# pierric/smart-chess-rust

Measured on AMD Instinct MI355X. Metric: MCTS simulations/sec (whole node), self-play rollout=180, at 1/2/4/8 MI355X, higher is better.
Workload: dtype bf16

## Files before the change

### smart-chess-rust_amd/csrc/mcts_kernels.hip

```cpp
#include "search_expand.hpp"

#include "launchers.hpp"

namespace sc {
__global__ __launch_bounds__(64) void k_debug_find_max(const float* u, int n, int* out) {
    const int lane = threadIdx.x;
    if (n <= 64) {
        const int r = wave_argmax_last_lane(lane < n ? u[lane] : 0.f, lane < n);
        if (lane == 0) out[0] = r;
    } else if (lane == 0) {
        out[0] = -2;
    }
    float best_u = 0.f;
    int best_i = -1;
#pragma unroll
    for (int r = 0; r < 4; r++) {
        const int i = lane + 64 * r;
        if (i < n) {
            const float v = u[i];
            if (best_i < 0 || v >= best_u) {
                best_u = v;
                best_i = i;
            }
        }
    }
    const int r4 = wave_argmax_last(best_u, best_i);
    if (lane == 0) out[1] = r4;
}

__global__ __launch_bounds__(64) void k_synth_eval(SpParams p) {
    const int g = blockIdx.x, lane = threadIdx.x;
    GameCtl& c = p.ctl[g];
    if (c.status != ST_ACTIVE || c.leaf_kind != LK_EVAL) return;
    const Position& pos = p.tpos[(size_t)g * p.tpos_cap + c.n_exp];
    uint64_t h = synth_pos_hash(pos) ^ p.synth_salt;
    int n = c.n_legal;
    const uint16_t* lm = p.legal_mv + (size_t)g * MAXC;
    if (p.evaluator == SYNTH_UNIFORM) {
        for (int i = lane; i < n; i += 64) p.prior[(size_t)g * MAXC + i] = 1.0f / (float)n;
        if (lane == 0) p.value[g] = 0.0f;
        return;
    }
    const bool coarse = p.evaluator == SYNTH_COARSE;
    unsigned long long sum = 0;
    for (int i = lane; i < n; i += 64) sum += coarse ? 1u + (synth_weight(h, lm[i]) >> 22) : synth_weight(h, lm[i]);
    sum = scw::wave_sum_u64(sum);
    float fs = (float)sum;
    for (int i = lane; i < n; i += 64)
        p.prior[(size_t)g * MAXC + i] = (float)(coarse ? 1u + (synth_weight(h, lm[i]) >> 22) : synth_weight(h, lm[i])) / fs;
    if (lane == 0) {
        const float v = synth_value(h);
        p.value[g] = coarse ? (v < -0.5f ? -0.5f : v >= 0.5f ? 0.5f : 0.0f) : v;
    }
}

__device__ inline int match_white(const SpParams& p, unsigned long long k) { return p.match_colours ? (int)(k & 1) : 0; }
__device__ inline unsigned long long match_ordinal(SpParams& p, int lane, int side) {
    const unsigned long long total = (unsigned long long)p.total_games;
    if (!p.match_colours && side) return total;
    unsigned long long n = 0;
    if (lane == 0) n = atomicAdd(&p.cnt->match_next[side], 1ULL);
    n = __shfl(n, 0, 64);
    const unsigned long long k = p.match_colours ? 2ULL * n + (unsigned long long)side : n;
    return k < total ? k : total;
}
__device__ inline int match_line_of(const SpParams& p, const MatchLines& ln, unsigned long long k) {
    return (int)((p.match_colours ? k >> 1 : k) % (unsigned long long)ln.n);
}
__device__ inline void match_copy_line(SpParams& p, int g, int lane, const Position* line, int len) {
    constexpr int W = (int)(sizeof(Position) / 8);
    static_assert(sizeof(Position) % 8 == 0, "a record is copied in 8-byte words");
    const unsigned long long* src = reinterpret_cast<const unsigned long long*>(line);
    unsigned long long* hist = reinterpret_cast<unsigned long long*>(p.hist + (size_t)g * p.hist_cap);
    unsigned long long* root = reinterpret_cast<unsigned long long*>(p.tpos + (size_t)g * p.tpos_cap);
    const int words = (len + 1) * W;
    wave_sync();
    for (int i = lane; i < words; i += 64) hist[i] = src[i];
    if (lane < W) root[lane] = src[len * W + lane];
    if (lane == 0) {
        p.ctl[g].ply = len;
        p.ctl[g].start_ply = len;
    }
}
__device__ inline void match_slot_start(SpParams& p, const MatchLines& ln, int g, int lane) {
    GameCtl& c = p.ctl[g];
    const int st = c.status, side = p.match_side & 1;
    const unsigned long long total = (unsigned long long)p.total_games;
    unsigned long long k;
    if (st == ST_MATCH_WAIT) {
        k = c.game_id - p.first_game_id;
    } else if (st == ST_IDLE) {
        k = match_ordinal(p, lane, side);
        if (k >= total) k = match_ordinal(p, lane, side ^ 1);
        if (k >= total) return;
    } else {
        return;
    }
    wave_sync();
    int len = 0;
    const Position* line = nullptr;
    if (ln.n > 0) {
        const int i = match_line_of(p, ln, k);
        const uint32_t a = ln.off[i], b = ln.off[i + 1];
        line = ln.tab + a;
        len = (int)(b - a) - 1;
    }
    if (side == (match_white(p, k) ^ (len & 1))) {
        try_start_game(p, g, lane, k);
        int now = 0;
        if (lane == 0) {
            now = c.status;
            if (now == ST_PENDING) c.status = ST_MATCH_WAIT;
        }
        if (len > 0 && __shfl(now, 0, 64) == ST_ACTIVE) match_copy_line(p, g, lane, line, len);
    } else if (lane == 0) {
        c.status = ST_MATCH_WAIT;
        c.leaf_kind = LK_NONE;
        c.game_id = p.first_game_id + k;
    }
}
__global__ __launch_bounds__(64) void k_match_boundary(SpParams p, MatchLines ln, int phase) {
    const int g = blockIdx.x, lane = threadIdx.x;
    if (phase == 1) {
        match_slot_start(p, ln, g, lane);
        return;
    }
    GameCtl& c = p.ctl[g];
    if (lane != 0 || c.status != ST_IDLE || c.trace_slot < 0) return;
    const TraceHdr& th = p.thdr[c.trace_slot];
    const int w = match_white(p, c.game_id - p.first_game_id);
    const int r = !th.has_outcome ? 3 : th.winner == 1 ? 0 : th.winner == 0 ? 1 : 2;
    p.match_tally()[((size_t)g * 2 + w) * 4 + r] += 1;
    c.trace_slot = -1;
}

__global__ __launch_bounds__(64) void k_init_slots(SpParams p, MatchLines ln) {
    const int g = blockIdx.x, lane = threadIdx.x;
    uint4* b = reinterpret_cast<uint4*>(p.boards + (size_t)g * 7168);
    for (int i = lane; i < 448; i += 64) b[i] = make_uint4(0, 0, 0, 0);
    if (lane < 8) p.meta[(size_t)g * 8 + lane] = 0;
    if (lane == 0) p.n_legal[g] = 0;
    if (p.match_recycle) {
        if (lane == 0) {
            p.ctl[g].status = ST_IDLE;
            p.ctl[g].leaf_kind = LK_NONE;
            p.ctl[g].trace_slot = -1;
        }
        wave_sync();
        match_slot_start(p, ln, g, lane);
        return;
    }
    if (g == 0 && lane == 0)
        atomicAdd(&p.cnt->next_game, (unsigned long long)(p.n_slots < p.total_games ? p.n_slots : p.total_games));
    if (g >= p.total_games) {
        if (lane == 0) {
            p.ctl[g].status = ST_IDLE;
            p.ctl[g].leaf_kind = LK_NONE;
        }
        return;
    }
    try_start_game(p, g, lane, (unsigned long long)g);
}

__global__ __launch_bounds__(64) void k_debug_choose_child(int n_cases, const int32_t* n_act, const int32_t* nc, const float* temperature,
                                                           const float* u, int tie_random, const float* w, const int32_t* w_off, int w_max,
                                                           int32_t* choice, float* total) {
    const int c = blockIdx.x, lane = threadIdx.x;
    if (c >= n_cases) return;
    float tot;
    const int ch = choose_child(n_act + (size_t)c * MAXC, uniform(nc[c]), temperature[c], u[c], tie_random, lane, w + uniform(w_off[c]), w_max, &tot);
    if (lane == 0) {
        choice[c] = ch;
        total[c] = tot;
    }
}

__global__ __launch_bounds__(64) void k_mcts(SpParams p, int do_expand, int do_select) {
    const int g = blockIdx.x, lane = threadIdx.x;
    __shared__ __attribute__((aligned(16))) int8_t s_stage[7168];
    __shared__ move_t s_moves[MAXC];
    __shared__ Position s_pos;
    __shared__ Position s_hist[8];
    __shared__ uint16_t s_ps[DEPTH_LDS];
    constexpr bool SC_ST = true;
    SC_STAMP(0);
    GameCtl cs_pre{};
    bool cs_pre_valid = false;
    if (do_expand) {
        dev_expand(p, g, lane, &s_pos, cs_pre, cs_pre_valid);
        __builtin_amdgcn_wave_barrier();
    }
    SC_STAMP(1);
    if (do_select) dev_select(p, g, lane, s_stage, s_moves, &s_pos, s_ps, s_hist, cs_pre, cs_pre_valid);
}

__global__ __launch_bounds__(64) void k_match_tally(const int32_t* tally, int n_slots, long long* out) {
    const int j = threadIdx.x;
    if (j >= 8) return;
    long long s = 0;
    for (int g = 0; g < n_slots; g++) s += tally[(size_t)g * 8 + j];
    out[j] = s;
}

__global__ __launch_bounds__(64) void k_open_lines(int n_lines, const uint16_t* moves, const uint32_t* move_off, Position* tab,
                                                   const uint32_t* rec_off, int32_t* status, Bases bases) {
    const int i = blockIdx.x, lane = threadIdx.x;
    if (i >= n_lines) return;
    __shared__ move_t s_moves[MAXC];
    __shared__ Position s_np;
    const uint16_t* mv = moves + move_off[i];
    const int nm = (int)(move_off[i + 1] - move_off[i]);
    const int pad = (int)(rec_off[i + 1] - rec_off[i]) - 1 - nm;
    Position* hist = tab + rec_off[i] + (pad > 0 ? pad : 0);
    Position cur = chain_start(bases, i, true);
    if (lane == 0) {
        Position none;
        set_startpos(none);
#pragma unroll
        for (int t = 0; t < 6; t++) none.pcs[t] = 0;
        none.occ[0] = none.occ[1] = 0;
        none.castling = 0;
        for (int k = 0; k < pad; k++) tab[rec_off[i] + k] = none;
        hist[0] = cur;
    }
    __syncthreads();
    int st;
    replay_checked(cur, mv, nm, hist, s_moves, &s_np, lane, st);
    if (st == 0) {
        int n = 0, winner = -1;
        gen_legal_wave(cur, s_moves, lane, n);
        __syncthreads();
        const HistChain hc{hist};
        if (outcome_claim_draw(hc, nm, &winner) != T_NONE || n == 0) st = 1;
    }
    if (lane == 0 && pad > 0) hist[0].flags = F_IRREV;
    if (lane == 0) status[i] = st;
}

__global__ __launch_bounds__(64) void k_set_position(SpParams p, int g, const uint16_t* moves, int n_moves, const Position* base) {
    const int lane = threadIdx.x;
    GameCtl& c = p.ctl[g];
    Position* hist = p.hist + (size_t)g * p.hist_cap;
    Position* tpos = p.tpos + (size_t)g * p.tpos_cap;
    __shared__ Position s_np;
    Position cur;
    if (base) {
        cur = uniform(*base);
    } else {
        set_startpos(cur);
        cur.key = position_key(cur);
    }
    if (lane == 0) hist[0] = cur;
    __syncthreads();
    for (int i = 0; i < n_moves && i + 1 < p.hist_cap; i++) replay_step(cur, moves[i], i, hist, tpos, &s_np, lane);
    if (lane == 0) {
        const size_t nb = (size_t)g * p.node_cap;
        tpos[0] = cur;
        p.N[nb] = 0;
        p.W[nb] = 0.0f;
        p.H[nb] = NodeHdr{-1, 0, 0};
        c.ply = n_moves;
        c.start_ply = n_moves;
        c.sim = 0;
        c.n_nodes = 1;
        c.n_exp = 1;
        c.leaf_kind = LK_NONE;
        c.rollout_cur = p.rollout;
        c.status = ST_ACTIVE;
    }
}

}

namespace scl {
void init_slots(const sc::SpParams& p, const sc::MatchLines& lines, hipStream_t s) {
    hipLaunchKernelGGL(sc::k_init_slots, dim3(p.n_slots), dim3(64), 0, s, p, lines);
}
void mcts(const sc::SpParams& p, int do_expand, int do_select, hipStream_t s) {
    hipLaunchKernelGGL(sc::k_mcts, dim3(p.n_slots), dim3(64), 0, s, p, do_expand, do_select);
}
void synth_eval(const sc::SpParams& p, hipStream_t s) { hipLaunchKernelGGL(sc::k_synth_eval, dim3(p.n_slots), dim3(64), 0, s, p); }
void debug_find_max(const float* d_u, int n, int* d_out, hipStream_t s) { hipLaunchKernelGGL(sc::k_debug_find_max, dim3(1), dim3(64), 0, s, d_u, n, d_out); }
void debug_choose_child(int n_cases, const int32_t* d_n_act, const int32_t* d_nc, const float* d_temperature, const float* d_u, int tie_random,
                        const float* d_w, const int32_t* d_w_off, int w_max, int32_t* d_choice, float* d_total, hipStream_t s) {
    if (n_cases <= 0) return;
    hipLaunchKernelGGL(sc::k_debug_choose_child, dim3(n_cases), dim3(64), 0, s, n_cases, d_n_act, d_nc, d_temperature, d_u, tie_random,
                       d_w, d_w_off, w_max, d_choice, d_total);
}
void match_boundary(const sc::SpParams& p, const sc::MatchLines& lines, hipStream_t s) {
    hipLaunchKernelGGL(sc::k_match_boundary, dim3(p.n_slots), dim3(64), 0, s, p, lines, 0);
    hipLaunchKernelGGL(sc::k_match_boundary, dim3(p.n_slots), dim3(64), 0, s, p, lines, 1);
}
void open_lines(int n_lines, const uint16_t* d_moves, const uint32_t* d_move_off, sc::Position* d_tab, const uint32_t* d_rec_off,
                int32_t* d_status, const sc::Bases& bases, hipStream_t s) {
    if (n_lines <= 0) return;
    hipLaunchKernelGGL(sc::k_open_lines, dim3(n_lines), dim3(64), 0, s, n_lines, d_moves, d_move_off, d_tab, d_rec_off, d_status, bases);
}
void match_tally(const int32_t* d_tally, int n_slots, long long* d_out, hipStream_t s) {
    hipLaunchKernelGGL(sc::k_match_tally, dim3(1), dim3(64), 0, s, d_tally, n_slots, d_out);
}
void set_position(const sc::SpParams& p, int slot, const uint16_t* d_moves, int n_moves, hipStream_t s, const sc::Position* d_base) {
    hipLaunchKernelGGL(sc::k_set_position, dim3(1), dim3(64), 0, s, p, slot, d_moves, n_moves, d_base);
}
}
```

### smart-chess-rust_amd/csrc/search_expand.hpp

```cpp
#pragma once
#include "search_select.hpp"
#include "value_tail.hpp"

namespace sc {
__device__ inline void try_start_game(SpParams& p, int g, int lane, unsigned long long k) {
    GameCtl& c = p.ctl[g];
    const int ts = (int)(k % (unsigned long long)p.trace_cap);
    const int st = p.thdr[ts].state;
    const unsigned long long prev_id = p.thdr[ts].game_id;
    bool ok;
    if (k < (unsigned long long)p.trace_cap) ok = st == TR_FREE;
    else ok = prev_id == p.first_game_id + k - (unsigned long long)p.trace_cap && (st == TR_FREE || (st == TR_DONE && !p.trace_hold));
    if (!ok) {
        if (lane == 0) {
            c.status = ST_PENDING;
            c.leaf_kind = LK_NONE;
            c.game_id = p.first_game_id + k;
        }
        return;
    }
    const size_t nb = (size_t)g * p.node_cap;
    if (lane == 0) {
        Position s;
        set_startpos(s);
        s.key = position_key(s);
        p.hist[(size_t)g * p.hist_cap] = s;
        p.tpos[(size_t)g * p.tpos_cap] = s;
        p.N[nb] = 0;
        p.W[nb] = 0.0f;
        p.P[nb] = 0.0f;
        p.U[nb] = 0.0f;
        p.MV[nb] = 0;
        p.H[nb] = NodeHdr{-1, 0, 0};
        c.status = ST_ACTIVE;
        c.ply = 0;
        c.start_ply = 0;
        c.sim = 0;
        c.n_nodes = 1;
        c.n_exp = 1;
        c.leaf = 0;
        c.path_len = 0;
        c.leaf_kind = LK_NONE;
        c.n_legal = 0;
        c.err = 0;
        c.rollout_cur = p.rollout;
        c.game_id = p.first_game_id + k;
        c.trace_slot = ts;
        TraceHdr& th = p.thdr[ts];
        th.n_steps = 0;
        th.has_outcome = 0;
        th.termination = 0;
        th.winner = -1;
        th.game_id = c.game_id;
        th.state = TR_LIVE;
    }
}
__device__ inline void start_new_game(SpParams& p, int g, int lane) {
    GameCtl& c = p.ctl[g];
    unsigned long long k = 0;
    if (lane == 0) k = atomicAdd(&p.cnt->next_game, 1ULL);
    k = __shfl(k, 0, 64);
    if (k >= (unsigned long long)p.total_games) {
        if (lane == 0) {
            c.status = ST_IDLE;
            c.leaf_kind = LK_NONE;
        }
        return;
    }
    try_start_game(p, g, lane, k);
}

__device__ inline void finish_game(SpParams& p, int g, int lane, int has_outcome, int term, int winner) {
    GameCtl& c = p.ctl[g];
    if (lane == 0) {
        TraceHdr& th = p.thdr[c.trace_slot];
        th.n_steps = c.ply - c.start_ply;
        th.has_outcome = has_outcome;
        th.termination = term;
        th.winner = winner;
        th.game_id = c.game_id;
        __threadfence();
        th.state = TR_DONE;
        atomicAdd(&p.cnt->games_finished, 1);
        c.status = ST_FINISHED;
    }
    wave_sync();
    start_new_game(p, g, lane);
}

__device__ inline int choose_child(const int32_t* n_act, int nc, float temperature, float u, int tie_random, int lane, const float* w,
                                   int w_max, float* total) {
    *total = 0.0f;
    if (temperature == 0.0f) {
        int bn = -1, bi = 0x7fffffff;
        for (int i = lane; i < nc; i += 64) {
            int n = n_act[i];
            if (n > bn) {
                bn = n;
                bi = i;
            }
        }
        for (int o = 32; o > 0; o >>= 1) {
            int on = __shfl_xor(bn, o, 64), oi = __shfl_xor(bi, o, 64);
            if (on > bn || (on == bn && oi < bi)) {
                bn = on;
                bi = oi;
            }
        }
        int choice = bi;
        if (tie_random) {
            int cnt = 0;
            for (int i = 0; i < nc; i++) cnt += n_act[i] == bn;
            int k = (int)(u * (float)cnt);
            if (k >= cnt) k = cnt - 1;
            for (int i = 0; i < nc; i++)
                if (n_act[i] == bn && k-- == 0) {
                    choice = i;
                    break;
                }
        }
        return choice;
    }
    const bool plain = 1.0f / temperature == 1.0f;
    auto weight = [&](int n) { return plain ? (float)n : w[n < w_max ? n : w_max]; };
    float sum = 0.0f;
    for (int i = 0; i < nc; i++) sum += weight(n_act[i]);
    *total = sum;
    float x = u * sum;
    float cum = 0.0f;
    int idx = 0;
    for (int i = 0; i < nc - 1; i++) {
        cum += weight(n_act[i]);
        if (cum <= x) idx++;
    }
    return idx;
}

using scvt::ValueTail;
__device__ __forceinline__ void value_tail_issue(const SpParams& p, int g, int lane, ValueTail& t) {
    const float* wf = p.vf_w;
    const int32_t* meta = p.meta + (size_t)g * 8;
#pragma unroll
    for (int k = 0; k < 7; k++) t.meta[k] = meta[k];
    const int j = 2 * lane;
    const float* vp = p.vpart + (size_t)g * 128 + j;
    const size_t vstride = (size_t)p.n_slots * 128;
#pragma unroll
    for (int ks = 0; ks < 32; ks++) t.acc[ks] = *reinterpret_cast<const float2*>(vp + (size_t)ks * vstride);
    if (p.vf_ksplit > 32) {
#pragma unroll
        for (int ks = 32; ks < 64; ks++) t.acc[ks] = *reinterpret_cast<const float2*>(vp + (size_t)ks * vstride);
    } else {
#pragma unroll
        for (int ks = 32; ks < 64; ks++) t.acc[ks] = make_float2(0.f, 0.f);
    }
    t.bias = *reinterpret_cast<const float2*>(wf + p.vf_fc1b + j);
    t.w2 = *reinterpret_cast<const float2*>(wf + p.vf_fc2w + j);
#pragma unroll
    for (int k = 0; k < 7; k++) t.wm[k] = *reinterpret_cast<const float2*>(wf + p.vf_fc1m + k * 128 + j);
    t.fc2b = wf[p.vf_fc2b];
}
__device__ __forceinline__ float value_tail_finish(const SpParams& p, const ValueTail& t) { return scvt::value_tail_compute(t, p.vf_ksplit); }

template <bool SC_ST = true>
__device__ __forceinline__ void dev_expand(SpParams& p, int g, int lane, Position* s_np_p, GameCtl& cs_out, bool& cs_valid) {
#pragma clang fp contract(off)
    Position& s_np = *s_np_p;
    GameCtl& c = p.ctl[g];
    {
        const void *a0 = p.ctl, *a1 = p.path, *a2 = p.prior, *a3 = p.legal_mv, *a4 = p.slot_cnt, *a5 = p.vpart, *a6 = p.vf_w, *a7 = p.meta;
        const int i0 = p.max_depth, i1 = p.vf_fused, i2 = p.n_slots, i3 = p.vf_ksplit;
        const uint32_t u0 = p.vf_fc1b, u1 = p.vf_fc1m, u2 = p.vf_fc2w, u3 = p.vf_fc2b;
        asm volatile("" ::"s"(a0), "s"(a1), "s"(a2), "s"(a3), "s"(a4), "s"(a5), "s"(a6), "s"(a7), "s"(i0), "s"(i1), "s"(i2), "s"(i3), "s"(u0), "s"(u1),
                     "s"(u2), "s"(u3));
    }
    const GameCtl craw = c;
    const int pth_raw = p.path[(size_t)g * p.max_depth + (lane < p.max_depth ? lane : p.max_depth - 1)];
    float prv[4];
    uint16_t lmv[4];
#pragma unroll
    for (int k = 0; k < 4; k++) {
        const int i = lane + 64 * k, ic = i < MAXC ? i : MAXC - 1;
        prv[k] = p.prior[(size_t)g * MAXC + ic];
        lmv[k] = p.legal_mv[(size_t)g * MAXC + ic];
    }
    const unsigned long long sc_sims = p.slot_cnt[(size_t)g * 2], sc_evals = p.slot_cnt[(size_t)g * 2 + 1];
    ValueTail vt;
    if (p.vf_fused) value_tail_issue(p, g, lane, vt);
    __builtin_amdgcn_sched_barrier(0);
    SC_XSTAMP(16);
    const GameCtl cs = uniform(craw);
    SC_XSTAMP(17);
    const int pth = lane < p.max_depth ? pth_raw : 0;
#pragma unroll
    for (int k = 0; k < 4; k++) {
        const int i = lane + 64 * k;
        prv[k] = i < MAXC ? prv[k] : 0.f;
        lmv[k] = i < MAXC ? lmv[k] : (uint16_t)0;
    }
    cs_out = cs;
    cs_valid = true;
    if (cs.status == ST_PENDING) {
        try_start_game(p, g, lane, cs.game_id - p.first_game_id);
        cs_valid = false;
        return;
    }
    if (cs.status != ST_ACTIVE || cs.leaf_kind == LK_NONE) return;
    const size_t nb = (size_t)g * p.node_cap;
    int32_t* N = p.N + nb;
    float* W = p.W + nb;
    float* P = p.P + nb;
    float* U = p.U + nb;
    uint16_t* MV = p.MV + nb;
    NodeHdr* H = p.H + nb;
    const int32_t* path = p.path + (size_t)g * p.max_depth;
    Position* hist = p.hist + (size_t)g * p.hist_cap;
    Position* tpos = p.tpos + (size_t)g * p.tpos_cap;

    const int leaf = cs.leaf, kind = cs.leaf_kind, plen = cs.path_len;
    float value = cs.leaf_value;
    int n_nodes = cs.n_nodes, n_exp = cs.n_exp;
    uint32_t err = 0;
    const bool inpath = lane < plen;
    int n0 = 0;
    float w0 = 0.f;
    if (inpath) {
        n0 = N[pth];
        w0 = W[pth];
    }
    if (kind == LK_EVAL) {
        value = p.vf_fused ? value_tail_finish(p, vt) : p.value[g];
        SC_XSTAMP(18);
        int n = cs.n_legal;
        if (n_nodes + n > p.node_cap || n_exp + 1 >= p.tpos_cap) {
            err = ERR_POOL_OVERFLOW;
        } else {
#pragma unroll
            for (int k = 0; k < 4; k++) {
                int i = lane + 64 * k;
                if (i < n) {
                    int id = n_nodes + i;
                    N[id] = 0;
                    W[id] = 0.0f;
                    P[id] = prv[k];
                    U[id] = 0.0f;
                    MV[id] = lmv[k];
                    H[id] = NodeHdr{-1, 0, 0};
                }
            }
            if (lane == 0) H[leaf] = NodeHdr{n_nodes, (uint16_t)n, (uint16_t)n_exp};
            n_nodes += n;
            n_exp += 1;
        }
    } else if (kind == LK_TERM_NEW) {
        if (lane == 0) H[leaf] = NodeHdr{value == 0.0f ? -2 : value > 0.0f ? -3 : -4, 0, 0};
    }
    SC_XSTAMP(19);
    if (inpath) {
        N[pth] = n0 + 1;
        W[pth] = w0 + value;
    }
    for (int d = lane + 64; d < plen; d += 64) {
        int nd = path[d];
        N[nd] += 1;
        W[nd] += value;
    }
    wave_sync();
    int sim = cs.sim + 1;
    if (lane == 0) {
        c.n_nodes = n_nodes;
        c.n_exp = n_exp;
        c.sim = sim;
        c.leaf_kind = LK_NONE;
        if (err) {
            c.err = cs.err | err;
            atomicOr(&p.cnt->err, (int)err);
        }
        p.slot_cnt[(size_t)g * 2] = sc_sims + 1ULL;
        if (kind == LK_EVAL) p.slot_cnt[(size_t)g * 2 + 1] = sc_evals + 1ULL;
    }
    SC_XSTAMP(20);
    cs_out.n_nodes = n_nodes;
    cs_out.n_exp = n_exp;
    cs_out.sim = sim;
    cs_out.leaf_kind = LK_NONE;
    cs_out.err = cs.err | err;
    const int budget = p.rollout_factor > 0.f ? cs.rollout_cur : p.rollout;
    if (sim < budget) return;
    cs_valid = false;

    wave_sync();
    const int ply = cs.ply;
    const NodeHdr h0 = H[0];
    const int nc = h0.nc, fc = h0.fc;
    if (nc == 0 || budget == 0) {
        HistChain hc{hist};
        int winner = -1;
        int term = outcome_claim_draw(hc, ply, &winner);
        finish_game(p, g, lane, term != T_NONE, term, winner);
        return;
    }
    const int ts = cs.trace_slot;
    const size_t tstep = (size_t)ts * p.num_steps + (size_t)(ply - cs.start_ply);
    for (int i = lane; i < nc; i += 64) {
        p.t_cmove[tstep * MAXC + i] = MV[fc + i];
        p.t_cn[tstep * MAXC + i] = N[fc + i];
        p.t_cq[tstep * MAXC + i] = W[fc + i];
        p.t_cu[tstep * MAXC + i] = U[fc + i];
    }
    const float temperature = (ply - cs.start_ply) < p.temp_switch ? 1.0f : p.temperature;
    const float u = (float)(sc_rng(p.seed, cs.game_id, (uint64_t)ply, 1, 0) >> 40) / 16777216.0f;
    float w_total;
    const int choice = choose_child(N + fc, nc, temperature, u, p.tie_random, lane, p.choice_w, p.choice_w_max, &w_total);
    move_t mv = MV[fc + choice];
    if (lane == 0) {
        p.t_move[tstep] = mv;
        p.t_q[tstep] = W[0];
        p.t_nchild[tstep] = nc;
    }
    Position np = uniform(hist[ply]);
    make_move(np, (move_t)uniform((int)mv));
    if (lane == 0) s_np = np;
    wave_sync();
    {
        DevChain ch{hist, ply, tpos, nullptr, &s_np, ply + 1};
        uint8_t rf = rep_flags_wave(ch, ply + 1, np.key, lane);
        np.flags = (uint8_t)((np.flags & F_IRREV) | rf);
    }
    wave_sync();
    if (lane == 0) {
        hist[ply + 1] = np;
        atomicAdd(&p.cnt->plies_done, 1ULL);
    }
    wave_sync();
    const int new_ply = ply + 1;
    if (lane == 0) c.ply = new_ply;
    const int i_step = ply - cs.start_ply;
    if (i_step > p.outcome_gate) {
        HistChain hc{hist};
        int winner = -1;
        int term = outcome_claim_draw(hc, new_ply, &winner);
        if (term != T_NONE) {
            wave_sync();
            finish_game(p, g, lane, 1, term, winner);
            return;
        }
    }
    if (i_step + 1 >= p.num_steps || new_ply + 1 >= p.hist_cap) {
        wave_sync();
        finish_game(p, g, lane, 0, 0, -1);
        return;
    }
    if (lane == 0) {
        tpos[0] = np;
        N[0] = 0;
        W[0] = 0.0f;
        P[0] = 0.0f;
        U[0] = 0.0f;
        MV[0] = mv;
        H[0] = NodeHdr{-1, 0, 0};
        c.n_nodes = 1;
        c.n_exp = 1;
        c.sim = 0;
    }
}

}
```

### smart-chess-rust_amd/csrc/search_select.hpp

```cpp
#pragma once
#include <type_traits>
#include <hip/hip_runtime.h>

#include "mcts_types.hpp"
#include "position_chain.hpp"

namespace sc {

using scw::dpp_i, scw::wave_sum_fixed, scw::wave_sum_i;

__device__ __forceinline__ int wave_argmax_last(float u, int idx) {
    unsigned b = __builtin_bit_cast(unsigned, u + 0.0f);
    unsigned key = (b & 0x80000000u) ? ~b : (b | 0x80000000u);
    int hi = idx >= 0 ? (int)key : 0, lo = idx;
    auto step = [&](int ohi, int olo) {
        const bool take = olo >= 0 && (lo < 0 || (unsigned)ohi > (unsigned)hi || ((unsigned)ohi == (unsigned)hi && olo > lo));
        hi = take ? ohi : hi;
        lo = take ? olo : lo;
    };
    step(dpp_i<0xB1>(hi), dpp_i<0xB1>(lo));
    step(dpp_i<0x4E>(hi), dpp_i<0x4E>(lo));
    step(dpp_i<0x141>(hi), dpp_i<0x141>(lo));
    step(dpp_i<0x140>(hi), dpp_i<0x140>(lo));
    int bh = __builtin_amdgcn_readlane(hi, 0), bl = __builtin_amdgcn_readlane(lo, 0);
#pragma unroll
    for (int r = 16; r < 64; r += 16) {
        const int oh = __builtin_amdgcn_readlane(hi, r), ol = __builtin_amdgcn_readlane(lo, r);
        const bool take = ol >= 0 && (bl < 0 || (unsigned)oh > (unsigned)bh || ((unsigned)oh == (unsigned)bh && ol > bl));
        bh = take ? oh : bh;
        bl = take ? ol : bl;
    }
    return bl;
}
__device__ __forceinline__ int wave_argmax_last_lane(float u, bool has) {
    unsigned b = __builtin_bit_cast(unsigned, u + 0.0f);
    unsigned key = (b & 0x80000000u) ? ~b : (b | 0x80000000u);
    int k = has ? (int)key : 0;
    auto umax = [](int a, int b2) { return (int)((unsigned)a > (unsigned)b2 ? (unsigned)a : (unsigned)b2); };
    int m = k;
    m = umax(m, dpp_i<0xB1>(m));
    m = umax(m, dpp_i<0x4E>(m));
    m = umax(m, dpp_i<0x141>(m));
    m = umax(m, dpp_i<0x140>(m));
    const int wm = umax(umax(__builtin_amdgcn_readlane(m, 0), __builtin_amdgcn_readlane(m, 16)),
                        umax(__builtin_amdgcn_readlane(m, 32), __builtin_amdgcn_readlane(m, 48)));
    const unsigned long long mask = __ballot(has && k == wm);
    return mask ? 63 - __clzll((long long)mask) : -1;
}
__device__ __forceinline__ NodeHdr uniform(const NodeHdr& q) {
    NodeHdr r;
    r.fc = uniform(q.fc);
    r.nc = (uint16_t)uniform((int)q.nc);
    r.ps = (uint16_t)uniform((int)q.ps);
    return r;
}
__device__ __forceinline__ GameCtl uniform(const GameCtl& q) {
    GameCtl r;
    r.status = uniform(q.status);
    r.ply = uniform(q.ply);
    r.sim = uniform(q.sim);
    r.n_nodes = uniform(q.n_nodes);
    r.n_exp = uniform(q.n_exp);
    r.leaf = uniform(q.leaf);
    r.path_len = uniform(q.path_len);
    r.leaf_kind = uniform(q.leaf_kind);
    r.n_legal = uniform(q.n_legal);
    r.leaf_value = __builtin_bit_cast(float, uniform(__builtin_bit_cast(int, q.leaf_value)));
    r.err = (uint32_t)uniform((int)q.err);
    r.trace_slot = uniform(q.trace_slot);
    r.game_id = uniform((bb_t)q.game_id);
    r.start_ply = uniform(q.start_ply);
    r.rollout_cur = uniform(q.rollout_cur);
    return r;
}

__device__ inline float u01_open(uint64_t& st) {
#pragma clang fp contract(off)
    st = mix64(st);
    return ((float)(st >> 40) + 0.5f) * (1.0f / 16777216.0f);
}
__device__ inline float gamma03(uint64_t st) {
#pragma clang fp contract(off)
    const float LN2 = 0.69314718f;
    const float alpha = 0.3f;
    const float boost = __builtin_amdgcn_exp2f(__builtin_amdgcn_logf(u01_open(st)) * (1.0f / alpha));
    const float d = alpha + 1.0f - 1.0f / 3.0f;
    const float c = 0.3390317518f;
    for (int it = 0; it < 64; it++) {
        float a = u01_open(st), b = u01_open(st);
        float x = __builtin_amdgcn_sqrtf(-2.0f * LN2 * __builtin_amdgcn_logf(a)) * __builtin_amdgcn_cosf(b);
        float v = 1.0f + c * x;
        if (v <= 0.0f) continue;
        v = v * v * v;
        float u = u01_open(st);
        if (LN2 * __builtin_amdgcn_logf(u) < 0.5f * x * x + d - d * v + d * (LN2 * __builtin_amdgcn_logf(v))) return boost * d * v;
    }
    return boost * d;
}

constexpr int DEPTH_LDS = 1024;

#ifdef SC_EXP
#define SC_XSTAMP(k) SC_STAMP(k)
#else
#define SC_XSTAMP(k)
#endif
#ifdef SC_EXP
#define SC_ST_DEFAULT true
#else
#define SC_ST_DEFAULT false
#endif
#define SC_STAMP(k)                                                                       \
    do {                                                                                  \
        if constexpr (SC_ST) {                                                            \
            if (p.dbg_cycles && lane == 0) p.dbg_cycles[(size_t)g * 32 + (k)] = clock64(); \
        }                                                                                 \
    } while (0)

struct HelperBox {
    int state, idx, root_ply, pad;
};
__device__ __forceinline__ void helper_post(HelperBox* box, int lane, int state, int idx, int root_ply) {
    if (!box) return;
    if (lane == 0) {
        box->idx = idx;
        box->root_ply = root_ply;
    }
    wave_sync();
    if (lane == 0) *reinterpret_cast<volatile int*>(&box->state) = state;
}
__device__ __forceinline__ void dev_encode_helper(const SpParams& p, int g, int lane, HelperBox* box, int8_t* s_stage, Position* s_leaf_p,
                                                  uint16_t* s_ps, Position* s_hist) {
    int st = 0;
    for (int spin = 0; spin < (1 << 22) && st == 0; spin++) {
        st = *reinterpret_cast<volatile int*>(&box->state);
        if (st == 0) __builtin_amdgcn_s_sleep(2);
    }
    st = __builtin_amdgcn_readfirstlane(st);
    if (st == 0 && lane == 0) atomicOr(&p.cnt->err, ERR_HELPER_TIMEOUT);
    if (st != 1 && st != 3) return;
    wave_sync();
    const int idx = __builtin_amdgcn_readfirstlane(box->idx), root_ply = __builtin_amdgcn_readfirstlane(box->root_ply);
    DevChain ch{p.hist + (size_t)g * p.hist_cap, root_ply, p.tpos + (size_t)g * p.tpos_cap, s_ps, s_leaf_p, idx};
    if (st == 3) {
        const bb_t key0 = s_leaf_p->key;
        const uint8_t rf = (uint8_t)__builtin_amdgcn_readfirstlane((int)rep_flags_wave(ch, idx, key0, lane));
        const uint8_t fl = (uint8_t)((s_leaf_p->flags & F_IRREV) | rf);
        wave_sync();
        if (lane == 0) {
            s_leaf_p->flags = fl;
            box->pad = fl;
        }
        wave_sync();
        if (lane == 0) *reinterpret_cast<volatile int*>(&box->state) = 4;
    }
    stage_history(ch, idx, lane, s_hist);
    wave_sync();
    encode_wave(s_hist, idx < 7 ? idx + 1 : 8, lane, s_stage, nullptr, p.meta + (size_t)g * 8);
}

template <bool PLANES_TO_HBM = true, bool SC_ST = true>
__device__ __forceinline__ bool dev_select(const SpParams& p, int g, int lane, int8_t* s_stage, move_t* s_moves, Position* s_leaf_p,
                                        uint16_t* s_ps, Position* s_hist, const GameCtl& cs_pre, bool cs_pre_valid,
                                        HelperBox* box = nullptr) {
#pragma clang fp contract(off)
    Position& s_leaf = *s_leaf_p;
    SC_STAMP(2);
    GameCtl& c = p.ctl[g];
    GameCtl cs = cs_pre;
    if (!cs_pre_valid) cs = uniform(c);
    const Position root_raw = p.tpos[(size_t)g * p.tpos_cap];
    const NodeHdr hdr_raw = p.H[(size_t)g * p.node_cap];
    const size_t nb0 = (size_t)g * p.node_cap + (1 + lane < p.node_cap ? 1 + lane : p.node_cap - 1);
    const int pf_n = p.N[nb0];
    const float pf_w = p.W[nb0], pf_p = p.P[nb0];
    const NodeHdr pf_h = p.H[nb0];
    __builtin_amdgcn_sched_barrier(0);
    const Position root = uniform(root_raw);
    NodeHdr hdr = uniform(hdr_raw);
    if (cs.status != ST_ACTIVE) {
        if (lane == 0) c.leaf_kind = LK_NONE;
        helper_post(box, lane, 2, 0, 0);
        return false;
    }
    const size_t nb = (size_t)g * p.node_cap;
    const int32_t* N = p.N + nb;
    const float* W = p.W + nb;
    const float* P = p.P + nb;
    float* U = p.U + nb;
    const uint16_t* MV = p.MV + nb;
    const NodeHdr* H = p.H + nb;
    int32_t* path = p.path + (size_t)g * p.max_depth;
    const Position* hist = p.hist + (size_t)g * p.hist_cap;
    Position* tpos = p.tpos + (size_t)g * p.tpos_cap;
    const int root_ply = cs.ply;
    const int root_turn = root.turn;
    const int dmax = p.max_depth < DEPTH_LDS ? p.max_depth : DEPTH_LDS;

    int node = 0, depth = 0, parent_ps = 0;
    if (lane == 0) {
        path[0] = 0;
        s_ps[0] = 0;
    }
    uint32_t err = 0;
    for (;;) {
        const int nc = hdr.nc;
        if (nc == 0) break;
        const int fc = hdr.fc;
        const int nr = (nc + 63) >> 6;
        int best_i = 0;
        NodeHdr nxt;
        auto level = [&](auto nrc) {
#pragma clang fp contract(off)
            constexpr int NRM = decltype(nrc)::value;
            int cn[NRM];
            float cw[NRM], cp[NRM];
            NodeHdr ch_[NRM];
#pragma unroll
            for (int r = 0; r < NRM; r++) {
                cn[r] = 0;
                cw[r] = 0.f;
                cp[r] = 0.f;
                ch_[r] = NodeHdr{-1, 0, 0};
                if (r < nr) {
                    int i = lane + 64 * r;
                    bool ok = i < nc;
                    if (r == 0 && depth == 0 && fc == 1) {
                        cn[0] = ok ? pf_n : 0;
                        cw[0] = ok ? pf_w : 0.f;
                        cp[0] = ok ? pf_p : 0.f;
                        ch_[0] = ok ? pf_h : NodeHdr{-1, 0, 0};
                    } else {
                        cn[r] = ok ? N[fc + i] : 0;
                        cw[r] = ok ? W[fc + i] : 0.f;
                        cp[r] = ok ? P[fc + i] : 0.f;
                        ch_[r] = ok ? H[fc + i] : NodeHdr{-1, 0, 0};
                    }
                }
            }
            if (nc > 1) {
                const bool reverse_q = ((root_turn ^ (depth & 1)) == BLACK);
                const bool noisy = depth == 0 && p.with_noise;
                float* nz = p.noise + (size_t)g * MAXC;
                float nzv[NRM];
#pragma unroll
                for (int r = 0; r < NRM; r++) nzv[r] = 0.f;
                if (noisy) {
                    if (!p.external_noise) {
                        float gsum = 0.0f;
#pragma unroll
                        for (int r = 0; r < NRM; r++) {
                            int i = lane + 64 * r;
                            if (i < nc) {
                                nzv[r] = gamma03(sc_rng(p.seed, cs.game_id, (uint64_t)root_ply, 3, (uint64_t)cs.sim * 256 + (uint64_t)i));
                                gsum += nzv[r];
                            }
                        }
                        gsum = wave_sum_fixed(gsum);
#pragma unroll
                        for (int r = 0; r < NRM; r++) {
                            int i = lane + 64 * r;
                            nzv[r] = nzv[r] / gsum;
                            if (i < nc) nz[i] = nzv[r];
                        }
                    } else {
#pragma unroll
                        for (int r = 0; r < NRM; r++) {
                            int i = lane + 64 * r;
                            if (i < nc) nzv[r] = nz[i];
                        }
                    }
                }
                int tot = 0;
#pragma unroll
                for (int r = 0; r < NRM; r++) tot += cn[r];
                tot = wave_sum_i(tot);
                const float sqrt_total = sqrtf((float)tot);
                float best_u = 0.0f;
                best_i = -1;
#pragma unroll
                for (int r = 0; r < NRM; r++) {
                    int i = lane + 64 * r;
                    if (r < nr && i < nc) {
                        float prior = cp[r];
                        if (noisy) prior = prior * (1.0f - p.epsilon) + nzv[r] * p.epsilon;
                        float average_award = cw[r] / ((float)cn[r] + 1e-4f) * (reverse_q ? -1.0f : 1.0f);
                        float exploration = (sqrt_total + 0.01f) / (1.0f + (float)cn[r]) * p.cpuct * prior;
                        float u = average_award + exploration;
                        U[fc + i] = u;
                        if (!isfinite(u)) err |= ERR_NONFINITE_UCT;
                        if (best_i < 0 || u >= best_u) {
                            best_u = u;
                            best_i = i;
                        }
                    }
                }
                if constexpr (NRM == 1) best_i = wave_argmax_last_lane(best_u, best_i >= 0);
                else best_i = wave_argmax_last(best_u, best_i);
            }
            best_i = __builtin_amdgcn_readfirstlane(best_i);
            const int rr = best_i >> 6;
            NodeHdr mine = ch_[0];
#pragma unroll
            for (int r = 1; r < NRM; r++)
                if (rr == r) mine = ch_[r];
            nxt.fc = __builtin_amdgcn_readlane(mine.fc, best_i & 63);
            int packed = __builtin_amdgcn_readlane((int)mine.nc | ((int)mine.ps << 16), best_i & 63);
            nxt.nc = (uint16_t)(packed & 0xffff);
            nxt.ps = (uint16_t)((unsigned)packed >> 16);
        };
        if (nr == 1) level(std::integral_constant<int, 1>{});
        else level(std::integral_constant<int, 4>{});
        parent_ps = hdr.ps;
        node = fc + best_i;
        hdr = nxt;
        depth++;
        if (depth >= dmax) {
            err |= ERR_DEPTH_OVERFLOW;
            depth--;
            break;
        }
        if (lane == 0) {
            path[depth] = node;
            s_ps[depth] = hdr.ps;
        }
    }
    SC_STAMP(3);
    if (p.dbg_cycles && lane == 0) p.dbg_cycles[(size_t)g * 32 + 7] = depth;
    unsigned long long anyerr = __ballot(err != 0);
    if (anyerr) {
        for (int o = 32; o > 0; o >>= 1) err |= __shfl_xor(err, o, 64);
        if (lane == 0) {
            c.err = cs.err | err;
            atomicOr(&p.cnt->err, (int)err);
        }
    }
    const int fcl = hdr.fc;
    if (lane == 0) {
        c.leaf = node;
        c.path_len = depth + 1;
    }
    if (fcl <= -2) {
        if (lane == 0) {
            c.leaf_kind = LK_TERM_CACHED;
            c.leaf_value = fcl == -2 ? 0.0f : fcl == -3 ? 1.0f : -1.0f;
            c.n_legal = 0;
        }
        helper_post(box, lane, 2, 0, 0);
        return false;
    }
    Position pos;
    if (depth == 0) {
        pos = root;
    } else {
        pos = uniform(tpos[parent_ps]);
        make_move(pos, (move_t)__builtin_amdgcn_readfirstlane((int)MV[node]));
    }
    if (lane == 0) s_leaf = pos;
    wave_sync();
    DevChain ch{hist, root_ply, tpos, s_ps, &s_leaf, root_ply + depth};
    const bool rep_by_helper = box && depth > 0;
    if (depth > 0 && !box) {
        uint8_t rf = (uint8_t)__builtin_amdgcn_readfirstlane((int)rep_flags_wave(ch, root_ply + depth, pos.key, lane));
        pos.flags = (uint8_t)((pos.flags & F_IRREV) | rf);
        wave_sync();
        if (lane == 0) s_leaf.flags = pos.flags;
        wave_sync();
    }
    SC_STAMP(4);
    if (box) helper_post(box, lane, rep_by_helper ? 3 : 1, root_ply + depth, root_ply);
    else stage_history(ch, root_ply + depth, lane, s_hist);
    if (lane == 0 && !rep_by_helper) tpos[cs.n_exp] = pos;
    int n = 0;
    bool in_check = gen_legal_wave(pos, s_moves, lane, n);
    wave_sync();
    SC_STAMP(5);
    if (depth == 0 && p.rollout_factor > 0.f && lane == 0) {
        const int r = (int)((float)n * p.rollout_factor);
        c.rollout_cur = r < 300 ? r : 300;
    }
    if (n == 0) {
        if (lane == 0) {
            c.leaf_kind = LK_TERM_NEW;
            c.leaf_value = in_check ? (pos.turn == WHITE ? -1.0f : 1.0f) : 0.0f;
            c.n_legal = 0;
        }
        return false;
    }
    uint16_t* lm = p.legal_mv + (size_t)g * MAXC;
    uint16_t* li = p.legal_idx + (size_t)g * MAXC;
    uint32_t bad = 0;
    for (int i = lane; i < n; i += 64) {
        move_t m = s_moves[i];
        int idx = move_index(m, pos.turn);
        if (idx < 0) {
            bad = 1;
            idx = 0;
        }
        lm[i] = m;
        li[i] = (uint16_t)idx;
    }
    if (__ballot(bad) && lane == 0) {
        c.err = cs.err | err | ERR_BAD_MOVE_INDEX;
        atomicOr(&p.cnt->err, ERR_BAD_MOVE_INDEX);
    }
    if (rep_by_helper) {
        int st = 3;
        for (int spin = 0; spin < (1 << 22) && st != 4; spin++) {
            st = *reinterpret_cast<volatile int*>(&box->state);
            if (st != 4) __builtin_amdgcn_s_sleep(1);
        }
        st = __builtin_amdgcn_readfirstlane(st);
        wave_sync();
        if (st != 4 && lane == 0) atomicOr(&p.cnt->err, ERR_HELPER_TIMEOUT);
        pos.flags = (uint8_t)__builtin_amdgcn_readfirstlane(box->pad);
        if (lane == 0) tpos[cs.n_exp] = pos;
    }
    const int idx = root_ply + depth;
    if (!box) encode_wave(s_hist, idx < 7 ? idx + 1 : 8, lane, s_stage, PLANES_TO_HBM ? p.boards + (size_t)g * 7168 : nullptr, p.meta + (size_t)g * 8);
    if (lane == 0) {
        c.leaf_kind = LK_EVAL;
        c.n_legal = n;
        p.n_legal[g] = n;
    }
    SC_STAMP(6);
    return true;
}

}
```

### smart-chess-rust_amd/csrc/step_kernels.hip

```cpp
#include "search_expand.hpp"
#include "nn_kernels.hpp"
#include "nn_tower32.hpp"

#include "launchers.hpp"
#include "tower_config.hpp"

namespace scstep {

__device__ __forceinline__ void fc1_tail(const scnn::TowerArgs& A, const sc::SpParams& p, const int g, const bool ran, scnn::Fc1Hand& fh) {
    const int tid = threadIdx.x, lane = tid & 63;
    const int wave = __builtin_amdgcn_readfirstlane(tid >> 6);
    const int mb = g >> 6, ks = g & 63;
    uint32_t* ctr = A.fc1_arrive + mb * 32;
#ifdef SC_EXP
#define TSTAMP(k) do { if (p.dbg_cycles && tid == 0) p.dbg_cycles[(size_t)g * 32 + 8 + (k)] = __builtin_amdgcn_s_memrealtime(); } while (0)
#else
#define TSTAMP(k)
#endif
    TSTAMP(0);
    if (!ran) {
        if (tid == 0) __hip_atomic_fetch_add(ctr, 1u, __ATOMIC_RELAXED, __HIP_MEMORY_SCOPE_AGENT);
        scnn::fc1_wload(fh.w, A.net, ks, 64, wave, lane);
        __builtin_amdgcn_sched_barrier(0);
    }
    const scnn::Fc1W& w = fh.w;
    const bool have_a = ran && fh.have_a;
#ifdef SC_EXP
    if (p.dbg_cycles && tid == 0) p.dbg_cycles[(size_t)g * 32 + 14] = have_a;
    if (have_a) { TSTAMP(1); TSTAMP(2); }
#endif
    if (tid == 0 && !have_a) {
        const uint64_t t0 = __builtin_amdgcn_s_memrealtime();
        uint32_t seen = ran ? fh.early : __hip_atomic_load(ctr, __ATOMIC_RELAXED, __HIP_MEMORY_SCOPE_AGENT);
        while ((int32_t)(seen - A.fc1_target) < 0) {
            __builtin_amdgcn_s_sleep(4);
            const uint64_t waited = __builtin_amdgcn_s_memrealtime() - t0;
            if (waited > 20000000ull) {
                atomicOr(&p.cnt->err, sc::ERR_HANDOFF_TIMEOUT);
                break;
            }
            if (waited > 100000ull && (__hip_atomic_load(&p.cnt->err, __ATOMIC_RELAXED, __HIP_MEMORY_SCOPE_AGENT) & sc::ERR_HANDOFF_TIMEOUT)) break;
            seen = __hip_atomic_load(ctr, __ATOMIC_RELAXED, __HIP_MEMORY_SCOPE_AGENT);
        }
        TSTAMP(1);
        if (A.fc1_acquire) __builtin_amdgcn_fence(__ATOMIC_ACQUIRE, "agent");
        asm volatile("s_waitcnt vmcnt(0)" ::: "memory");
        TSTAMP(2);
    }
    __syncthreads();
    scnn::bf16_t* s_a = reinterpret_cast<scnn::bf16_t*>(scnn::g_smem);
    if (!have_a) scnn::fc1_load_a(fh.a, A.hval, mb, ks, tid);
    scnn::fc1_put_a(s_a, fh.a, tid);
    __syncthreads();
    TSTAMP(3);
    scnn::fc1_mma_store(w, s_a, A.vpart, A.n_pos, mb, ks, 64, wave, lane);
    TSTAMP(4);
#ifdef SC_EXP
    asm volatile("s_waitcnt vmcnt(0)" ::: "memory");
    TSTAMP(5);
#endif
}

template <class P, int C, int RS, int TPI, int AB, bool STAMPS = false>
__global__ __launch_bounds__(256, 1) void k_step(scnn::TowerArgs A, sc::SpParams p, int do_expand) {
    __shared__ __attribute__((aligned(16))) int8_t s_stage[7168];
    __shared__ sc::move_t s_moves[sc::MAXC];
    __shared__ sc::Position s_pos;
    __shared__ sc::Position s_hist[8];
    __shared__ uint16_t s_ps[sc::DEPTH_LDS];
    __shared__ sc::HelperBox s_box;
    const int g = blockIdx.x;
    const int lane = threadIdx.x & 63;
#ifdef SC_EXP
    const long long t_entry = clock64();
#endif
    scnn::kernarg_prefetch<sizeof(scnn::TowerArgs) + sizeof(sc::SpParams) + sizeof(int)>();
#ifdef SC_EXP
    if (p.dbg_cycles && threadIdx.x == 0) p.dbg_cycles[(size_t)g * 32 + 21] = t_entry;
#endif
#define PHASE_STAMP(k, cond) do { if constexpr (STAMPS) { if (p.dbg_cycles && (cond)) p.dbg_cycles[(size_t)g * 32 + (k)] = __builtin_amdgcn_s_memrealtime(); } } while (0)
    PHASE_STAMP(24, threadIdx.x == 0);
    if (threadIdx.x == 0) s_box.state = 0;
    __syncthreads();
    auto search = [&](int wave) -> bool {
        if (wave == 1) {
            sc::dev_encode_helper(p, g, lane, &s_box, s_stage, &s_pos, s_ps, s_hist);
            return true;
        }
        constexpr bool SC_ST = STAMPS || SC_ST_DEFAULT;
        SC_STAMP(0);
        sc::GameCtl cs_pre{};
        bool cs_pre_valid = false;
        if (do_expand) {
            sc::dev_expand<SC_ST>(p, g, lane, &s_pos, cs_pre, cs_pre_valid);
            __builtin_amdgcn_wave_barrier();
        }
        SC_STAMP(1);
        const bool need_net = sc::dev_select<false, SC_ST>(p, g, lane, s_stage, s_moves, &s_pos, s_ps, s_hist, cs_pre, cs_pre_valid, &s_box);
        PHASE_STAMP(25, lane == 0);
        return need_net;
    };
    scnn::Fc1Hand fh;
    const bool ran = scnn::tower_body<P, C, RS, TPI, AB>(A, g, s_stage, search, fh);
    PHASE_STAMP(26, threadIdx.x == 0);
    if (A.fc1_arrive) fc1_tail(A, p, g, ran, fh);
    PHASE_STAMP(27, threadIdx.x == 0);
#undef PHASE_STAMP
}

}

namespace scl {
#define K_STEP(P, C, RS, TPI, AB) scstep::k_step<scnn::P, C, RS, TPI, AB>
#define K_STEP_STAMPED scstep::k_step<scnn::PrecBF16, 128, SC_T32_RS, SC_T32_TPI, SC_T32_AB, true>
const char* step_init() {
    const void* kn[4] = {reinterpret_cast<const void*>(&K_STEP(PrecBF16, 128, SC_T32_RS, SC_T32_TPI, SC_T32_AB)),
                         reinterpret_cast<const void*>(&K_STEP(PrecBF16, 256, SC_T32W_RS, SC_T32W_TPI, SC_T32W_AB)),
                         reinterpret_cast<const void*>(&K_STEP(PrecFP8, 128, SC_T8_RS, SC_T8_TPI, SC_T8_AB)),
                         reinterpret_cast<const void*>(&K_STEP(PrecFP8, 256, SC_T8W_RS, SC_T8W_TPI, SC_T8W_AB))};
    for (int i = 0; i < 4; i++) {
        hipError_t e = hipFuncSetAttribute(kn[i], hipFuncAttributeMaxDynamicSharedMemorySize, scnn::tower32_lds_bytes(i & 1 ? 256 : 128, i >= 2 && i < 4));
        if (e != hipSuccess) return hipGetErrorString(e);
    }
    {
        hipError_t e = hipFuncSetAttribute(reinterpret_cast<const void*>(&K_STEP_STAMPED), hipFuncAttributeMaxDynamicSharedMemorySize, scnn::tower32_lds_bytes(128));
        if (e != hipSuccess) return hipGetErrorString(e);
    }
    return nullptr;
}
int step_blocks_per_cu(const scnn::NetLayout& net) {
    int n = 0;
    hipError_t e;
    if (net.fp8 && net.C == 128)
        e = hipOccupancyMaxActiveBlocksPerMultiprocessor(&n, K_STEP(PrecFP8, 128, SC_T8_RS, SC_T8_TPI, SC_T8_AB), 256, scnn::tower32_lds_bytes(128, true));
    else if (net.fp8)
        e = hipOccupancyMaxActiveBlocksPerMultiprocessor(&n, K_STEP(PrecFP8, 256, SC_T8W_RS, SC_T8W_TPI, SC_T8W_AB), 256, scnn::tower32_lds_bytes(256, true));
    else if (net.C == 128)
        e = hipOccupancyMaxActiveBlocksPerMultiprocessor(&n, K_STEP(PrecBF16, 128, SC_T32_RS, SC_T32_TPI, SC_T32_AB), 256, scnn::tower32_lds_bytes(128));
    else
        e = hipOccupancyMaxActiveBlocksPerMultiprocessor(&n, K_STEP(PrecBF16, 256, SC_T32W_RS, SC_T32W_TPI, SC_T32W_AB), 256, scnn::tower32_lds_bytes(256));
    return e == hipSuccess && n > 0 ? n : 1;
}
void step(const scnn::TowerArgs& a, const sc::SpParams& p, int do_expand, hipStream_t s) {
    const dim3 grid(p.n_slots), block(256);
    if (a.net.fp8 && a.net.C == 128)
        hipLaunchKernelGGL((K_STEP(PrecFP8, 128, SC_T8_RS, SC_T8_TPI, SC_T8_AB)), grid, block, scnn::tower32_lds_bytes(128, true), s, a, p, do_expand);
    else if (a.net.fp8)
        hipLaunchKernelGGL((K_STEP(PrecFP8, 256, SC_T8W_RS, SC_T8W_TPI, SC_T8W_AB)), grid, block, scnn::tower32_lds_bytes(256, true), s, a, p, do_expand);
    else if (a.net.C == 128 && p.dbg_cycles)
        hipLaunchKernelGGL((K_STEP_STAMPED), grid, block, scnn::tower32_lds_bytes(128), s, a, p, do_expand);
    else if (a.net.C == 128)
        hipLaunchKernelGGL((K_STEP(PrecBF16, 128, SC_T32_RS, SC_T32_TPI, SC_T32_AB)), grid, block, scnn::tower32_lds_bytes(128), s, a, p, do_expand);
    else
        hipLaunchKernelGGL((K_STEP(PrecBF16, 256, SC_T32W_RS, SC_T32W_TPI, SC_T32W_AB)), grid, block, scnn::tower32_lds_bytes(256), s, a, p, do_expand);
}
}
```

Measured before the change: 2.299 million.

## Prefetch root stats in expand and offload root Dirichlet noise to helper wave

Issues the root header and child N/W/P/H loads early inside expand and patches them with the just-applied backup so select can reuse them without reloading. A helper wave precomputes the gamma noise for the first 64 root children in parallel and posts it through a shared box, so the search wave skips those RNG evaluations. This adds spin-wait synchronisation, a larger LDS helper box, and a stale-prefetch correctness risk if the patching misses a case, such as the root position now being reloaded from tpos when depth is zero.

Result: no change. 2.303 million, median of 3 (+0.2%).

```diff
diff --git a/smart-chess-rust_amd/csrc/mcts_kernels.hip b/smart-chess-rust_amd/csrc/mcts_kernels.hip
--- a/smart-chess-rust_amd/csrc/mcts_kernels.hip
+++ b/smart-chess-rust_amd/csrc/mcts_kernels.hip
@@ -186,12 +186,13 @@
     SC_STAMP(0);
     GameCtl cs_pre{};
     bool cs_pre_valid = false;
+    RootPre rp_pre{};
     if (do_expand) {
-        dev_expand(p, g, lane, &s_pos, cs_pre, cs_pre_valid);
+        dev_expand(p, g, lane, &s_pos, cs_pre, cs_pre_valid, rp_pre);
         __builtin_amdgcn_wave_barrier();
     }
     SC_STAMP(1);
-    if (do_select) dev_select(p, g, lane, s_stage, s_moves, &s_pos, s_ps, s_hist, cs_pre, cs_pre_valid);
+    if (do_select) dev_select(p, g, lane, s_stage, s_moves, &s_pos, s_ps, s_hist, cs_pre, cs_pre_valid, rp_pre);
 }
 
 __global__ __launch_bounds__(64) void k_match_tally(const int32_t* tally, int n_slots, long long* out) {
diff --git a/smart-chess-rust_amd/csrc/search_expand.hpp b/smart-chess-rust_amd/csrc/search_expand.hpp
--- a/smart-chess-rust_amd/csrc/search_expand.hpp
+++ b/smart-chess-rust_amd/csrc/search_expand.hpp
@@ -163,7 +163,7 @@
 __device__ __forceinline__ float value_tail_finish(const SpParams& p, const ValueTail& t) { return scvt::value_tail_compute(t, p.vf_ksplit); }
 
 template <bool SC_ST = true>
-__device__ __forceinline__ void dev_expand(SpParams& p, int g, int lane, Position* s_np_p, GameCtl& cs_out, bool& cs_valid) {
+__device__ __forceinline__ void dev_expand(SpParams& p, int g, int lane, Position* s_np_p, GameCtl& cs_out, bool& cs_valid, RootPre& rp_out) {
 #pragma clang fp contract(off)
     Position& s_np = *s_np_p;
     GameCtl& c = p.ctl[g];
@@ -176,6 +176,7 @@
     }
     const GameCtl craw = c;
     const int pth_raw = p.path[(size_t)g * p.max_depth + (lane < p.max_depth ? lane : p.max_depth - 1)];
+    rp_out.valid = false;
     float prv[4];
     uint16_t lmv[4];
 #pragma unroll
@@ -222,12 +223,15 @@
     int n_nodes = cs.n_nodes, n_exp = cs.n_exp;
     uint32_t err = 0;
     const bool inpath = lane < plen;
+    RootPre rp = root_pre_issue(p, g, lane);
     int n0 = 0;
     float w0 = 0.f;
     if (inpath) {
         n0 = N[pth];
         w0 = W[pth];
     }
+    NodeHdr leaf_h{-1, 0, 0};
+    bool leaf_h_new = false;
     if (kind == LK_EVAL) {
         value = p.vf_fused ? value_tail_finish(p, vt) : p.value[g];
         SC_XSTAMP(18);
@@ -235,6 +239,8 @@
         if (n_nodes + n > p.node_cap || n_exp + 1 >= p.tpos_cap) {
             err = ERR_POOL_OVERFLOW;
         } else {
+            leaf_h = NodeHdr{n_nodes, (uint16_t)n, (uint16_t)n_exp};
+            leaf_h_new = true;
 #pragma unroll
             for (int k = 0; k < 4; k++) {
                 int i = lane + 64 * k;
@@ -248,14 +254,17 @@
                     H[id] = NodeHdr{-1, 0, 0};
                 }
             }
-            if (lane == 0) H[leaf] = NodeHdr{n_nodes, (uint16_t)n, (uint16_t)n_exp};
+            if (lane == 0) H[leaf] = leaf_h;
             n_nodes += n;
             n_exp += 1;
         }
     } else if (kind == LK_TERM_NEW) {
-        if (lane == 0) H[leaf] = NodeHdr{value == 0.0f ? -2 : value > 0.0f ? -3 : -4, 0, 0};
+        leaf_h = NodeHdr{value == 0.0f ? -2 : value > 0.0f ? -3 : -4, 0, 0};
+        leaf_h_new = true;
+        if (lane == 0) H[leaf] = leaf_h;
     }
     SC_XSTAMP(19);
+    asm volatile("" : "+v"(n0), "+v"(w0));
     if (inpath) {
         N[pth] = n0 + 1;
         W[pth] = w0 + value;
@@ -286,7 +295,19 @@
     cs_out.leaf_kind = LK_NONE;
     cs_out.err = cs.err | err;
     const int budget = p.rollout_factor > 0.f ? cs.rollout_cur : p.rollout;
-    if (sim < budget) return;
+    if (sim < budget) {
+        if (plen >= 2 && uniform(rp.hdr.fc) == 1) {
+            const int c1 = __builtin_amdgcn_readlane(pth, 1) - 1;
+            if (lane == c1) {
+                rp.pf_n = rp.pf_n + 1;
+                rp.pf_w = rp.pf_w + value;
+            }
+            if (leaf_h_new && leaf >= 1 && leaf <= (int)rp.hdr.nc && lane == leaf - 1) rp.pf_h = leaf_h;
+            rp.valid = true;
+            rp_out = rp;
+        }
+        return;
+    }
     cs_valid = false;
 
     wave_sync();
diff --git a/smart-chess-rust_amd/csrc/search_select.hpp b/smart-chess-rust_amd/csrc/search_select.hpp
--- a/smart-chess-rust_amd/csrc/search_select.hpp
+++ b/smart-chess-rust_amd/csrc/search_select.hpp
@@ -119,6 +119,9 @@
 
 struct HelperBox {
     int state, idx, root_ply, pad;
+    int nz_state, nz_ply, nz_sim, nz_pad;
+    uint64_t nz_gid;
+    float nz_raw[64];
 };
 __device__ __forceinline__ void helper_post(HelperBox* box, int lane, int state, int idx, int root_ply) {
     if (!box) return;
@@ -129,8 +132,44 @@
     wave_sync();
     if (lane == 0) *reinterpret_cast<volatile int*>(&box->state) = state;
 }
+__device__ __forceinline__ void dev_noise_helper(const SpParams& p, int g, int lane, HelperBox* box, int do_expand) {
+#pragma clang fp contract(off)
+    if (!p.with_noise || p.external_noise) return;
+    const GameCtl cs = uniform(p.ctl[g]);
+    int sim = cs.sim;
+    bool draw = cs.status == ST_ACTIVE;
+    if (do_expand && cs.leaf_kind != LK_NONE) {
+        sim += 1;
+        draw = draw && sim < (p.rollout_factor > 0.f ? cs.rollout_cur : p.rollout);
+    }
+    if (draw) {
+        box->nz_raw[lane] = gamma03(sc_rng(p.seed, cs.game_id, (uint64_t)cs.ply, 3, (uint64_t)sim * 256 + (uint64_t)lane));
+        if (lane == 0) {
+            box->nz_gid = cs.game_id;
+            box->nz_ply = cs.ply;
+            box->nz_sim = sim;
+        }
+    }
+    wave_sync();
+    if (lane == 0) *reinterpret_cast<volatile int*>(&box->nz_state) = draw ? 1 : 2;
+}
+__device__ __forceinline__ bool noise_from_helper(HelperBox* box, int lane, uint64_t game_id, int ply, int sim, float& raw) {
+    int st = 0;
+    for (int spin = 0; spin < (1 << 16) && st == 0; spin++) {
+        st = *reinterpret_cast<volatile int*>(&box->nz_state);
+        if (st == 0) __builtin_amdgcn_s_sleep(1);
+    }
+    st = __builtin_amdgcn_readfirstlane(st);
+    wave_sync();
+    if (st != 1) return false;
+    if (uniform(box->nz_gid) != game_id || uniform(box->nz_ply) != ply || uniform(box->nz_sim) != sim) return false;
+    raw = box->nz_raw[lane];
+    return true;
+}
+
 __device__ __forceinline__ void dev_encode_helper(const SpParams& p, int g, int lane, HelperBox* box, int8_t* s_stage, Position* s_leaf_p,
-                                                  uint16_t* s_ps, Position* s_hist) {
+                                                  uint16_t* s_ps, Position* s_hist, int do_expand) {
+    dev_noise_helper(p, g, lane, box, do_expand);
     int st = 0;
     for (int spin = 0; spin < (1 << 22) && st == 0; spin++) {
         st = *reinterpret_cast<volatile int*>(&box->state);
@@ -159,9 +198,30 @@
     encode_wave(s_hist, idx < 7 ? idx + 1 : 8, lane, s_stage, nullptr, p.meta + (size_t)g * 8);
 }
 
+struct RootPre {
+    int turn;
+    NodeHdr hdr;
+    int pf_n;
+    float pf_w, pf_p;
+    NodeHdr pf_h;
+    bool valid;
+};
+__device__ __forceinline__ RootPre root_pre_issue(const SpParams& p, int g, int lane) {
+    RootPre r;
+    r.turn = p.tpos[(size_t)g * p.tpos_cap].turn;
+    r.hdr = p.H[(size_t)g * p.node_cap];
+    const size_t nb0 = (size_t)g * p.node_cap + (1 + lane < p.node_cap ? 1 + lane : p.node_cap - 1);
+    r.pf_n = p.N[nb0];
+    r.pf_w = p.W[nb0];
+    r.pf_p = p.P[nb0];
+    r.pf_h = p.H[nb0];
+    r.valid = false;
+    return r;
+}
+
 template <bool PLANES_TO_HBM = true, bool SC_ST = true>
 __device__ __forceinline__ bool dev_select(const SpParams& p, int g, int lane, int8_t* s_stage, move_t* s_moves, Position* s_leaf_p,
-                                        uint16_t* s_ps, Position* s_hist, const GameCtl& cs_pre, bool cs_pre_valid,
+                                        uint16_t* s_ps, Position* s_hist, const GameCtl& cs_pre, bool cs_pre_valid, const RootPre& rp_pre,
                                         HelperBox* box = nullptr) {
 #pragma clang fp contract(off)
     Position& s_leaf = *s_leaf_p;
@@ -169,15 +229,15 @@
     GameCtl& c = p.ctl[g];
     GameCtl cs = cs_pre;
     if (!cs_pre_valid) cs = uniform(c);
-    const Position root_raw = p.tpos[(size_t)g * p.tpos_cap];
-    const NodeHdr hdr_raw = p.H[(size_t)g * p.node_cap];
-    const size_t nb0 = (size_t)g * p.node_cap + (1 + lane < p.node_cap ? 1 + lane : p.node_cap - 1);
-    const int pf_n = p.N[nb0];
-    const float pf_w = p.W[nb0], pf_p = p.P[nb0];
-    const NodeHdr pf_h = p.H[nb0];
-    __builtin_amdgcn_sched_barrier(0);
-    const Position root = uniform(root_raw);
-    NodeHdr hdr = uniform(hdr_raw);
+    RootPre rp = rp_pre;
+    if (!rp.valid) {
+        rp = root_pre_issue(p, g, lane);
+        __builtin_amdgcn_sched_barrier(0);
+    }
+    const int pf_n = rp.pf_n;
+    const float pf_w = rp.pf_w, pf_p = rp.pf_p;
+    const NodeHdr pf_h = rp.pf_h;
+    NodeHdr hdr = uniform(rp.hdr);
     if (cs.status != ST_ACTIVE) {
         if (lane == 0) c.leaf_kind = LK_NONE;
         helper_post(box, lane, 2, 0, 0);
@@ -194,7 +254,7 @@
     const Position* hist = p.hist + (size_t)g * p.hist_cap;
     Position* tpos = p.tpos + (size_t)g * p.tpos_cap;
     const int root_ply = cs.ply;
-    const int root_turn = root.turn;
+    const int root_turn = uniform(rp.turn);
     const int dmax = p.max_depth < DEPTH_LDS ? p.max_depth : DEPTH_LDS;
 
     int node = 0, depth = 0, parent_ps = 0;
@@ -248,11 +308,14 @@
                 if (noisy) {
                     if (!p.external_noise) {
                         float gsum = 0.0f;
+                        float raw0 = 0.f;
+                        const bool have0 = box && noise_from_helper(box, lane, cs.game_id, root_ply, cs.sim, raw0);
 #pragma unroll
                         for (int r = 0; r < NRM; r++) {
                             int i = lane + 64 * r;
                             if (i < nc) {
-                                nzv[r] = gamma03(sc_rng(p.seed, cs.game_id, (uint64_t)root_ply, 3, (uint64_t)cs.sim * 256 + (uint64_t)i));
+                                if (r == 0 && have0) nzv[r] = raw0;
+                                else nzv[r] = gamma03(sc_rng(p.seed, cs.game_id, (uint64_t)root_ply, 3, (uint64_t)cs.sim * 256 + (uint64_t)i));
                                 gsum += nzv[r];
                             }
                         }
@@ -351,7 +414,7 @@
     }
     Position pos;
     if (depth == 0) {
-        pos = root;
+        pos = uniform(tpos[0]);
     } else {
         pos = uniform(tpos[parent_ps]);
         make_move(pos, (move_t)__builtin_amdgcn_readfirstlane((int)MV[node]));
diff --git a/smart-chess-rust_amd/csrc/step_kernels.hip b/smart-chess-rust_amd/csrc/step_kernels.hip
--- a/smart-chess-rust_amd/csrc/step_kernels.hip
+++ b/smart-chess-rust_amd/csrc/step_kernels.hip
@@ -80,23 +80,24 @@
 #endif
 #define PHASE_STAMP(k, cond) do { if constexpr (STAMPS) { if (p.dbg_cycles && (cond)) p.dbg_cycles[(size_t)g * 32 + (k)] = __builtin_amdgcn_s_memrealtime(); } } while (0)
     PHASE_STAMP(24, threadIdx.x == 0);
-    if (threadIdx.x == 0) s_box.state = 0;
+    if (threadIdx.x == 0) s_box.state = s_box.nz_state = 0;
     __syncthreads();
     auto search = [&](int wave) -> bool {
         if (wave == 1) {
-            sc::dev_encode_helper(p, g, lane, &s_box, s_stage, &s_pos, s_ps, s_hist);
+            sc::dev_encode_helper(p, g, lane, &s_box, s_stage, &s_pos, s_ps, s_hist, do_expand);
             return true;
         }
         constexpr bool SC_ST = STAMPS || SC_ST_DEFAULT;
         SC_STAMP(0);
         sc::GameCtl cs_pre{};
         bool cs_pre_valid = false;
+        sc::RootPre rp_pre{};
         if (do_expand) {
-            sc::dev_expand<SC_ST>(p, g, lane, &s_pos, cs_pre, cs_pre_valid);
+            sc::dev_expand<SC_ST>(p, g, lane, &s_pos, cs_pre, cs_pre_valid, rp_pre);
             __builtin_amdgcn_wave_barrier();
         }
         SC_STAMP(1);
-        const bool need_net = sc::dev_select<false, SC_ST>(p, g, lane, s_stage, s_moves, &s_pos, s_ps, s_hist, cs_pre, cs_pre_valid, &s_box);
+        const bool need_net = sc::dev_select<false, SC_ST>(p, g, lane, s_stage, s_moves, &s_pos, s_ps, s_hist, cs_pre, cs_pre_valid, rp_pre, &s_box);
         PHASE_STAMP(25, lane == 0);
         return need_net;
     };
```
